# anonymous-author-918/deq-mpc-corl

Measured on AMD Instinct MI355X. Metric: QP solves/sec at (B,T=20,nx=13,nu=4), higher is better.
Workload: dtype f32

## Files before the change

### deq-mpc-corl_amd/_lib.py

```python
from __future__ import annotations

import ctypes as C
import os

_HERE = os.path.dirname(os.path.abspath(__file__))
LIB_PATH = os.environ.get("MI_ALQP_LIB") or os.path.join(_HERE, "csrc", "libmi_alqp.so")

ABI_VERSION = 16


class AlqpDims(C.Structure):
    _fields_ = [("B", C.c_int), ("T", C.c_int), ("nx", C.c_int), ("nu", C.c_int)]


class AlqpParams(C.Structure):
    _fields_ = [("al_iter", C.c_int), ("max_newton", C.c_int), ("n_ls", C.c_int),
                ("flags", C.c_int), ("rho_scale", C.c_double), ("variant", C.c_int),
                ("skip_flag", C.c_void_p), ("exit_tol", C.c_double), ("newton_counts", C.c_void_p),
                ("exit_scratch", C.c_void_p), ("quad_stagger", C.c_int)]


class AlqpTrace(C.Structure):
    _fields_ = [("g", C.c_void_p), ("d", C.c_void_p), ("phi", C.c_void_p),
                ("phi_prev", C.c_void_p), ("k", C.c_void_p), ("accept", C.c_void_p)]


class AlqpObstacles(C.Structure):
    _fields_ = [("pos", C.c_void_p), ("radius", C.c_double), ("nobs", C.c_int), ("state_estimator", C.c_int)]


class AlqpBwdDyn(C.Structure):
    _fields_ = [("lam", C.c_void_p), ("sb_lam", C.c_long), ("dF", C.c_void_p), ("dc", C.c_void_p), ("dx0", C.c_void_p)]


class AlqpIpmParams(C.Structure):
    _fields_ = [("flags", C.c_int), ("max_iter", C.c_int), ("iter0", C.c_int), ("kkt_eps", C.c_double),
                ("variant", C.c_int)]


class AlqpRigidParams(C.Structure):
    _fields_ = [("mass", C.c_double), ("J", C.c_double * 9), ("Jinv", C.c_double * 9), ("g", C.c_double * 3),
                ("motor_dist", C.c_double), ("kf", C.c_double), ("bf", C.c_double), ("km", C.c_double),
                ("act_scale", C.c_double), ("u_hover", C.c_double), ("pend_L", C.c_double), ("ss", C.c_double * 12),
                ("bf_force", C.c_double)]


IPM_VARIANTS = {"auto": 0, "generic_lds": 1, "generic_ws": 2, "resident": 3}


ALQP_IPM_INIT, ALQP_IPM_RESID, ALQP_IPM_STEP, ALQP_IPM_LOOP, ALQP_IPM_FINAL = 1, 2, 4, 8, 16
ALQP_INIT_MERIT = 1
ALQP_DUAL_UPDATE = 2
ALQP_SAVE_FACTOR = 4
ALQP_WS_PRIMED = 8
ALQP_EXIT_IN_KERNEL = 16
ALQP_E_COOP = -4
VARIANT_AUTO, VARIANT_TEAM, VARIANT_QUAD = 0, 1, 2

ERRORS = {-1: "bad argument", -2: "unsupported (nx, nu), or horizon / batch beyond what the requested kernel can hold or address",
          -3: "kernel launch failed", -4: "grid too large for a cooperative launch"}

_P = C.c_void_p
_SIGS = {
    "alqp_solve_nonlin": (C.c_int, [C.POINTER(AlqpDims), C.POINTER(AlqpParams), C.c_int, C.c_double, _P, _P, _P, _P, _P,
                                    C.c_long, C.c_long, _P, _P, _P, _P, _P, _P, _P, _P, C.c_size_t, _P]),
    "alqp_dyn_pendulum1l": (C.c_int, [C.c_long, _P, _P, C.c_double, _P, _P, _P, _P]),
    "alqp_dyn_cartpole1l": (C.c_int, [C.c_long, _P, _P, C.c_double, _P, _P, _P, _P]),
    "alqp_dyn_cartpole1l_v2": (C.c_int, [C.c_long, _P, _P, C.c_double, _P, _P, _P, _P]),
    "alqp_dyn_cartpole2l": (C.c_int, [C.c_long, _P, _P, C.c_double, _P, _P, _P, _P]),
    "alqp_dyn_rexquadrotor": (C.c_int, [C.c_long, C.POINTER(AlqpRigidParams), _P, _P, C.c_double, _P, _P, _P]),
    "alqp_dyn_flyingcartpole": (C.c_int, [C.c_long, C.POINTER(AlqpRigidParams), _P, _P, C.c_double, _P, _P, _P]),
    "alqp_solve_lin": (C.c_int, [C.POINTER(AlqpDims), C.POINTER(AlqpParams), _P, _P, _P, _P, _P, _P, _P,
                                 C.c_long, C.c_long, _P, _P, _P, _P, _P, _P, _P, _P,
                                 C.POINTER(AlqpTrace), _P, C.c_size_t, _P]),
    "alqp_solve_lin_shared": (C.c_int, [C.POINTER(AlqpDims), C.POINTER(AlqpParams), _P, _P, _P, _P,
                                        C.c_long, C.c_long, C.c_long, C.c_long, _P, _P, _P,
                                        C.c_long, C.c_long, _P, _P, _P, _P, _P, _P, _P, _P,
                                        C.POINTER(AlqpTrace), _P, C.c_size_t, _P]),
    "alqp_solve_lin_dense": (C.c_int, [C.POINTER(AlqpDims), C.POINTER(AlqpParams), _P, _P, _P, _P, _P, _P, _P,
                                       C.c_long, C.c_long, _P, _P, _P, _P, _P, _P, _P, _P,
                                       C.POINTER(AlqpTrace), _P]),
    "alqp_solve_lin_xbox": (C.c_int, [C.POINTER(AlqpDims), C.POINTER(AlqpParams), _P, _P, _P, _P, _P, _P, _P,
                                      C.c_long, C.c_long, _P, _P, C.c_long, C.c_long, _P, _P, _P, _P, _P, _P, _P, _P,
                                      C.POINTER(AlqpTrace), _P]),
    "alqp_solve_lin_poly": (C.c_int, [C.POINTER(AlqpDims), C.POINTER(AlqpParams), _P, _P, _P, _P, _P, _P, _P,
                                      C.c_long, C.c_long, _P, _P, C.c_int, C.c_long, C.c_long, C.c_long, C.c_long,
                                      _P, _P, _P, _P, _P, _P, _P, _P, C.POINTER(AlqpTrace), _P]),
    "alqp_newton_step": (C.c_int, [C.POINTER(AlqpDims), _P, _P, _P, _P, _P, _P, _P, _P, _P, _P,
                                   C.c_long, C.c_long, C.POINTER(AlqpObstacles), _P, C.c_size_t, _P, _P, _P, _P, _P]),
    "alqp_merit": (C.c_int, [C.POINTER(AlqpDims), C.c_int, _P, _P, _P, _P, _P, _P, _P, _P, _P,
                             C.c_long, C.c_long, C.POINTER(AlqpObstacles), _P, _P, _P]),
    "alqp_linesearch_pick": (C.c_int, [C.POINTER(AlqpDims), C.c_int, _P, _P, _P, _P, _P, _P, _P]),
    "alqp_dual_update": (C.c_int, [C.POINTER(AlqpDims), _P, _P, _P, _P, _P, C.c_long, C.c_long,
                                   C.POINTER(AlqpObstacles), _P, _P, C.c_double, _P]),
    "alqp_backward": (C.c_int, [C.POINTER(AlqpDims), _P, _P, C.c_size_t, _P, _P, _P, _P, _P, _P,
                                C.POINTER(AlqpBwdDyn), _P]),
    "alqp_merit_pick": (C.c_int, [C.POINTER(AlqpDims), C.c_int, _P, _P, _P, _P, _P, _P, _P, _P, _P,
                                  C.c_long, C.c_long, C.POINTER(AlqpObstacles), _P, _P, _P, _P, _P, _P, _P]),
    "alqp_ipm_solve": (C.c_int, [C.POINTER(AlqpDims), C.POINTER(AlqpIpmParams), _P, _P, _P, _P, _P, _P, _P,
                                 C.c_long, C.c_long, C.c_long, C.c_long, C.c_long, C.c_long, _P, C.c_size_t, _P,
                                 _P, _P, _P, _P, _P, _P, _P, _P, _P, _P]),
    "alqp_ipm_backward": (C.c_int, [C.POINTER(AlqpDims), _P, _P, C.c_long, C.c_long, C.c_long, C.c_long, _P, _P, _P,
                                    _P, C.c_size_t, _P, _P, _P, _P, C.c_int, _P]),
}
_PLAIN = {
    "alqp_abi_version": (C.c_int, []),
    "alqp_supported": (C.c_int, [C.POINTER(AlqpDims), C.c_int]),
    "alqp_supported_variant": (C.c_int, [C.POINTER(AlqpDims), C.c_int, C.c_int]),
# ... 42 lines not shown
```

### deq-mpc-corl_amd/backend.py

```python
from __future__ import annotations

import ctypes as C

import os

import torch

from . import _lib


def _dt(t):
    if t.dtype == torch.float32:
        return "f32"
    if t.dtype == torch.float64:
        return "f64"
    raise TypeError(f"mi_alqp: unsupported dtype {t.dtype}")


def _ptr(t, name, dtype=None, allow_none=False):
    if t is None:
        if allow_none:
            return None
        raise ValueError(f"mi_alqp: {name} is required")
    if not t.is_cuda:
        raise RuntimeError(
            f"mi_alqp: {name} lives on {t.device}; the solver only runs on a ROCm device "
            "(no CPU fallback)")
    if not t.is_contiguous():
        raise ValueError(f"mi_alqp: {name} must be contiguous")
    if dtype is not None and t.dtype != dtype:
        raise TypeError(f"mi_alqp: {name} has dtype {t.dtype}, expected {dtype}")
    return C.c_void_p(t.data_ptr())


def _stream():
    return C.c_void_p(torch.cuda.current_stream().cuda_stream)


_DEBUG_FLAGS = ((int(os.environ.get("ALQP_DEBUG_STAGGER", "0")) & 0xff) << 24) | ((int(os.environ.get("ALQP_DEBUG_STAGGER_CU", "0")) & 0xf) << 20)


class DynGrads:

    __slots__ = ("lam", "dF", "dc", "dx0")

    def __init__(self, lam=None, dF=None, dc=None, dx0=None):
        self.lam, self.dF, self.dc, self.dx0 = lam, dF, dc, dx0


def _dyn_args(dyn, dims, dt):
    if dyn is None:
        return None
    B, T, nx, nu = dims
    lam = dyn.lam
    if lam is None:
        if dyn.dF is not None:
            raise ValueError("mi_alqp: dyn.dF needs dyn.lam (the multipliers the solve returned)")
        lam_p, sb = None, 0
    else:
        if (not lam.is_cuda or lam.dtype != dt or lam.dim() != 2 or lam.shape[0] != B or lam.shape[1] < (T - 1) * nx
                or lam.stride(1) != 1 or (B > 1 and lam.stride(0) < (T - 1) * nx)):
            raise ValueError(f"mi_alqp: dyn.lam must be a [B, >= (T-1) nx] {dt} device tensor with unit inner stride")
        lam_p, sb = lam.data_ptr(), max(int(lam.stride(0)), (T - 1) * nx)
    outs = []
    for t, name, shape in ((dyn.dF, "dF", (B, T - 1, nx, nx + nu)), (dyn.dc, "dc", (B, T - 1, nx)),
                           (dyn.dx0, "dx0", (B, nx))):
        if t is not None and tuple(t.shape) != shape:
            raise ValueError(f"mi_alqp: dyn.{name} has shape {tuple(t.shape)}, expected {shape}")
        outs.append(None if t is None else _ptr(t, "dyn." + name, dt).value)
    return _lib.AlqpBwdDyn(lam_p, sb, *outs)


def _step_length(h, K, dt):
    if not torch.is_tensor(h):
        return float(h), None
    hpt = h.to(dt).reshape(-1).contiguous()
    if hpt.numel() != K:
        raise ValueError("mi_alqp: h must be a number or one value per point")
    return 0.0, hpt


class HipBackend:

    name = "hip"
    supports_exit_in_kernel = True
    default_variant = "auto"
    QUAD_MIN_BATCH = 4096

    def __init__(self):
        self.lib = _lib.load()
        self._ws = {}
        if os.environ.get("ALQP_QUAD_STAGGER") is not None:
# ... 520 lines not shown
```

### deq-mpc-corl_amd/csrc/alqp_quad.hip

```cpp
#if defined(ALQP_BWD_DYN_UNIT) || defined(ALQP_SHDYN_UNIT)
#undef ALQP_PHASE_TIMING
#endif
#include <hip/hip_runtime.h>

#include "alqp_quad.hpp"
#include "alqp_dims.hpp"
#include "alqp_launch.hpp"

#if defined(ALQP_QUAD_F32) == defined(ALQP_QUAD_F64)
#error "compile alqp_quad.hip with exactly one of -DALQP_QUAD_F32, -DALQP_QUAD_F64"
#endif

namespace alqp {

#ifndef ALQP_FUSE_LS
#define ALQP_FUSE_LS 1
#endif
#ifdef ALQP_PHASE_TIMING
__device__ unsigned long long g_phase_cycles[10];
#define QSTAMP(b) qd.stamp(b)
#else
#define QSTAMP(b)
#endif
#ifdef ALQP_SHDYN_UNIT
// ... 18 lines not shown
        int stag = a.stagger;
        const int mode = (a.flags >> 20) & 0xf;
        if ((a.flags >> 24) & 0xff) stag = (a.flags >> 24) & 0xff;
        if (stag > 0) {
            const unsigned hw = __builtin_amdgcn_s_getreg(4 | (0 << 6) | (31 << 11));
            int simd = (hw >> 4) & 3;
            if (mode == 1) simd = simd * 16 + ((hw >> 8) & 0xf);
            if (mode == 2) simd &= 1;
            if (mode == 3) simd = blockIdx.x & 1;
            if (mode == 4) simd = (simd & 1) ^ (blockIdx.x & 1);
            if (mode == 5) simd = (hw >> 8) & 3;
            for (int i = 0; i < simd * stag; ++i) __builtin_amdgcn_s_sleep(16);
        }
    }
#ifdef ALQP_ALIAS_ALL
    const int b = (active ? b_raw : a.B - 1) % ALQP_ALIAS_ALL;
#else
    const int b = active ? b_raw : a.B - 1;
#endif
    const int T = a.T, M = C::M(T);

    Quad<real, NX, NU> qd;
    __shared__ real w_lds[QCfg<real, NX, NU>::WLDS_WORDS];
    qd.wl = w_lds + threadIdx.x;
    qd.q = lane & 3;
    qd.T = T;
    qd.active = active;
    qd.gQd = a.Qd + (size_t)b * T * N;
    qd.gq = a.q + (size_t)b * T * N;
#ifdef ALQP_SHDYN_UNIT
    qd.gF = a.F + (size_t)b * a.sb_F;
    qd.gc = a.c + (size_t)b * a.sb_c;
    qd.mt_F = a.mt_F; qd.mt_c = a.mt_c;
#else
    qd.gF = a.F + (size_t)b * (T - 1) * NX * N;
    qd.gc = a.c + (size_t)b * (T - 1) * NX;
#endif
    qd.gx0 = a.x0 + (size_t)b * NX;
    qd.gulo = a.ulo + (size_t)b * a.sb_u;
    qd.guhi = a.uhi + (size_t)b * a.sb_u;
    qd.st_u = a.st_u;
    qd.gz = a.z + (size_t)b * T * N;
    qd.glam = a.lam + (size_t)b * M;
    qd.rec = ws + C::rec_base(b, T);
    qd.gFw = const_cast<real *>(qd.gF);
    qd.dyn_h = a.dyn_h;
    qd.rho = a.rho[b];
    qd.info = 0;
    real phi_prev = a.phi[b];
#ifdef ALQP_PHASE_TIMING
    for (int i = 0; i < 10; ++i) qd.tacc[i] = 0;
#endif
    QSTAMP(-1);
    if (!(a.flags & ALQP_WS_PRIMED)) {
        if constexpr (NL) qd.stage_in(false, false);
        else qd.stage_in(a.max_newton == 0 || a.al_iter == 0 || (a.flags & ALQP_EXIT_IN_KERNEL) ||
                         (!C::PHI0_FWD && (a.flags & ALQP_INIT_MERIT)));
    }
    const bool ref_exit = (a.flags & ALQP_EXIT_IN_KERNEL) != 0;
    int gphase = 0;

    int step_id = 0;
    bool pend = false;
    real alpha_pend = 0;
    int bad = 0;
    real rn2 = 0, phi_next = 0;
    for (int it = 0; it < a.al_iter; ++it) {
        bool phi_from_forward = false;
        if (a.flags & ALQP_INIT_MERIT) {
            if (it > 0) {
                phi_prev = phi_next;
            } else if (C::PHI0_FWD && a.max_newton > 0 && !ref_exit) {
                phi_from_forward = true;
            } else {
                if constexpr (NL) qd.template linearize<Dyn>(real(0), false);
                real p1[1];
                qd.template merit_candidates<1>(p1, true);
                phi_prev = p1[0];
            }
        }
        pend = false;
        double nrm_old = 0;
        int n_done = 0;
        if (ref_exit) {
            int bad0 = 0;
            const real r0 = it == 0 ? qd.rplus2(bad0) : rn2;
            nrm_old = sqrt(grid_sum_ordered(wave_sum_leaders(exit_term(r0, qor(qd.info)), active && qd.q == 0), a.exit_scratch, gphase));
        }
        for (int st = 0; st < a.max_newton; ++st, ++step_id) {
            real *tg = nullptr;
            if constexpr (TRACE) tg = (tr.g && active) ? tr.g + ((size_t)step_id * a.B + b) * T * N : nullptr;
            QSTAMP(9);
            if constexpr (NL) {
                qd.template linearize<Dyn>(alpha_pend, pend);
                pend = false;
            }
            qd.forward(tg, alpha_pend, pend, (phi_from_forward && st == 0) ? &phi_prev : nullptr);
            real ph[20];
            qd.template backward<FUSE_LS>(ph);
            QSTAMP(-1);
            if constexpr (TRACE) {
                if (tr.d && active) {
                    real *td = tr.d + ((size_t)step_id * a.B + b) * T * N;
                    for (int t = 0; t < T; ++t)
                        for (int j = qd.q; j < N; j += 4) td[t * N + j] = qd.recp(t)[C::wn(C::oY, j)];
                }
            }
            if constexpr (NL) qd.template merit_nonlin<Dyn>(ph);
            else if constexpr (!FUSE_LS) qd.template merit_candidates<20>(ph, false);
            QSTAMP(6);
            int kbest = 0;
            real best = ph[0];
#pragma unroll
            for (int k = 1; k < 20; ++k) {
                if (k < a.n_ls && !(best != best) && (ph[k] != ph[k] || ph[k] < best)) {
                    best = ph[k];
                    kbest = k;
                }
            }
            const bool acc = best < phi_prev;
            if constexpr (TRACE) {
                if (active && qd.q == 0) {
                    if (tr.phi)
#pragma unroll
                        for (int k = 0; k < 20; ++k)
                            if (k < a.n_ls) tr.phi[((size_t)step_id * a.n_ls + k) * a.B + b] = ph[k];
                    if (tr.phi_prev) tr.phi_prev[(size_t)step_id * a.B + b] = phi_prev;
                    if (tr.k) tr.k[(size_t)step_id * a.B + b] = kbest;
                    if (tr.accept) tr.accept[(size_t)step_id * a.B + b] = acc ? 1 : 0;
                }
            }
            const real alpha = acc ? real(1) / real(1 << kbest) : real(0);
            pend = true;
            alpha_pend = alpha;
            QSTAMP(7);
            phi_prev = best;
            if (ref_exit) {
                int bad1 = 0;
                real ph_unused = 0, r1 = 0;
                qd.template iter_end<Dyn>(alpha_pend, pend, false, (real)a.rho_scale, false, ph_unused, r1, bad1);
                pend = false;
                const double nw = sqrt(grid_sum_ordered(wave_sum_leaders(exit_term(r1, qor(qd.info)), active && qd.q == 0), a.exit_scratch, gphase));
                ++n_done;
                if (nw < a.exit_tol || fabs(nrm_old - nw) / nw < a.exit_tol) break;
                nrm_old = nw;
            }
        }
        if (ref_exit && a.newton_counts && blockIdx.x == 0 && lane == 0) a.newton_counts[it] = grid_barrier_timed_out(a.exit_scratch) ? -1 : n_done;
        bad = 0;
        qd.template iter_end<Dyn>(alpha_pend, pend, (a.flags & ALQP_DUAL_UPDATE) != 0, (real)a.rho_scale, it + 1 == a.al_iter,
                    phi_next, rn2, bad);
        pend = false;
    }
    if (a.al_iter <= 0) {
        rn2 = qd.rplus2(bad);
        qd.stage_out();
    }
#ifdef ALQP_PHASE_TIMING
    QSTAMP(9);
    if (lane == 0)
        for (int i = 0; i < 10; ++i) atomicAdd(&g_phase_cycles[i], qd.tacc[i]);
#endif
    if (active && qd.q == 0) {
        a.rho[b] = qd.rho;
        a.phi[b] = phi_prev;
        if (a.rnorm2) a.rnorm2[b] = rn2;
        if (a.info && qd.info && a.info[b] == 0) a.info[b] = qd.info;
        if (a.status) a.status[b] = bad ? 0 : 1;
    }
}

template <typename real, int NX, int NU, bool DYN = false>
__global__ __launch_bounds__(64) __attribute__((amdgpu_waves_per_eu(1, 1))) void k_backward_quad(BwdArgs<real, DYN> a, real *ws) {
    using C = QCfg<real, NX, NU>;
    constexpr int N = C::N;
    const int lane = threadIdx.x, qi = lane >> 2;
    const int b_raw = blockIdx.x * 16 + qi;
    const bool active = b_raw < a.B;
    const int b = active ? b_raw : a.B - 1;
    const int T = a.T;
    Quad<real, NX, NU> qd;
    __shared__ real w_lds[QCfg<real, NX, NU>::WLDS_WORDS];
    qd.wl = w_lds + threadIdx.x;
    qd.q = lane & 3;
    qd.T = T;
    qd.active = active;
    qd.gF = a.F + (size_t)b * (T - 1) * NX * N;
    qd.gQd = nullptr; qd.gq = nullptr; qd.gc = nullptr; qd.gx0 = nullptr; qd.gulo = nullptr; qd.guhi = nullptr;
    qd.st_u = 0;
    qd.gz = nullptr; qd.glam = nullptr;
    qd.rec = ws + C::rec_base(b, T);
    qd.rho = a.rho[b];
    qd.info = 0;
    qd.solve_forward(a.gbar + (size_t)b * T * N);
    real unused[20];
    qd.template backward<false>(unused);
    if (active) {
        const real *zf = a.z_final + (size_t)b * T * N;
        real *qg = a.q_grad + (size_t)b * T * N;
        real *Qg = a.Qd_grad + (size_t)b * T * N;
        for (int t = 0; t < T; ++t)
// ... 182 lines not shown
```

### deq-mpc-corl_amd/csrc/alqp_quad.hpp

```cpp
#pragma once
#include <hip/hip_runtime.h>

#include <type_traits>

#include "alqp_team.hpp"
#include "alqp_dyn.hpp"

namespace alqp {

template <int Q>
__device__ inline float qb(float v) {
    return __builtin_bit_cast(float, __builtin_amdgcn_mov_dpp(__builtin_bit_cast(int, v), Q * 0x55, 0xF, 0xF, true));
}
template <int Q>
__device__ inline double qb(double v) {
    long long b = __builtin_bit_cast(long long, v);
    int lo = __builtin_amdgcn_mov_dpp((int)(b & 0xffffffffll), Q * 0x55, 0xF, 0xF, true);
    int hi = __builtin_amdgcn_mov_dpp((int)(b >> 32), Q * 0x55, 0xF, 0xF, true);
    return __builtin_bit_cast(double, ((long long)hi << 32) | (unsigned int)lo);
}
template <typename real>
__device__ inline real qbv(real v, int src) {
    switch (src & 3) {
        case 0: return qb<0>(v);
// ... 42 lines not shown
}
__device__ inline void gst4(float *p, float a, float b, float c, float d) {
    f4u t; t.x = a; t.y = b; t.z = c; t.w = d;
    *reinterpret_cast<f4u *>(p) = t;
}
__device__ inline void gst4(double *p, double a, double b, double c, double d) {
    d4u t; t.x = a; t.y = b; t.z = c; t.w = d;
    *reinterpret_cast<d4u *>(p) = t;
}
template <int LEN, typename real>
__device__ inline void gload(const real *p, real (&dst)[LEN]) {
#pragma unroll
    for (int c = 0; c + 4 <= LEN; c += 4) gld4(p + c, dst[c], dst[c + 1], dst[c + 2], dst[c + 3]);
#pragma unroll
    for (int c = (LEN / 4) * 4; c < LEN; ++c) dst[c] = p[c];
}

#ifndef ALQP_W_LDS
#define ALQP_W_LDS 1
#endif
#ifndef ALQP_EXP_NOQ
#define ALQP_EXP_NOQ 0
#endif
#ifndef ALQP_EXP_NORS
#define ALQP_EXP_NORS 0
#endif
#ifndef ALQP_EXP_NOL
#define ALQP_EXP_NOL 0
#endif
template <typename real, int SW, int N, bool IN_LDS>
struct WPanel {
    real a[SW][N];
    __device__ __forceinline__ real (&operator[](int s))[N] { return a[s]; }
    __device__ __forceinline__ const real (&operator[](int s) const)[N] { return a[s]; }
};
template <typename real, int N>
struct WRowLds {
    real *p;
    __device__ __forceinline__ real &operator[](int k) const { return p[k * 64]; }
};
template <typename real, int SW, int N>
struct WPanel<real, SW, N, true> {
    real *base;
    __device__ __forceinline__ WRowLds<real, N> operator[](int s) const { return WRowLds<real, N>{base + s * N * 64}; }
};
template <int LEN, typename real>
__device__ __forceinline__ void gload(const real *p, WRowLds<real, LEN> row) {
    real tmp[LEN];
    gload<LEN>(p, tmp);
#pragma unroll
    for (int k = 0; k < LEN; ++k) row[k] = tmp[k];
}

struct NoDyn {
    static constexpr int ID = 0;
};

struct Fld {
    int h, t;
};
template <int H, int T>
struct FldT {
    static constexpr int h = H, t = T;
    __host__ __device__ constexpr operator Fld() const { return {H, T}; }
};
template <typename real>
struct FRef {
    real *p;
    Fld f;
};
template <typename real, int H, int T>
__device__ __forceinline__ FRef<std::remove_const_t<real>> operator+(real *p, FldT<H, T>) {
    return {const_cast<std::remove_const_t<real> *>(p), Fld{H, T}};
}

template <typename real, int NX_, int NU_>
struct QCfg {
    static constexpr int NX = NX_, NU = NU_, N = NX_ + NU_;
    static constexpr int SH = (N + 3) / 4;
    static constexpr int SW = (NX + 3) / 4;
    static constexpr int SY = SH;
    static constexpr int HT = 2 * SH * (SH + 1);
    __host__ __device__ static constexpr int hidx(int s, int j) { return 2 * s * (s + 1) + j; }
    static constexpr int ST = 2 * SW * (SW + 1);
    static constexpr int BLK = 64 / (int)sizeof(real);
#ifndef ALQP_REC_IL_F32
#define ALQP_REC_IL_F32 2
#endif
    static constexpr int IL = sizeof(real) == 4 ? ALQP_REC_IL_F32 : 1;
    static_assert(IL == 1 || BLK == 16, "groups of 16 words are 64-byte blocks");
    __host__ __device__ static constexpr int w(int x) { return (x / 16) * (16 * IL) + x % 16; }
    static constexpr int NLAST = N - 4 * (SH - 1);
    __host__ __device__ static constexpr int lanes_of(int s) { return s == SH - 1 ? NLAST : 4; }
    __host__ __device__ static constexpr int lstride(int s) { return lanes_of(s) == 3 ? 16 : 4 * lanes_of(s); }
    __host__ __device__ static constexpr int lbase(int s) {
        int o = 0;
        for (int i = 0; i < s; ++i) o += (i + 1) * lstride(i);
        return o;
    }
    static constexpr int LW = lbase(SH);
    static constexpr bool PHI0_FWD = sizeof(real) == 4;
#ifndef ALQP_S_AFTER_F32
#define ALQP_S_AFTER_F32 0
#endif
    static constexpr bool S_AFTER = sizeof(real) == 8 || ALQP_S_AFTER_F32;
#ifndef ALQP_W_LDS_F32
// ... 399 lines not shown
        const real a0 = sel4(real(1), real(0.5), real(0.25), real(0.125), q);
        for (int t = 0; t < T; ++t) {
            const bool dyn = t < T - 1;
            const real *rp = recp(t), *rn = recp(dyn ? t + 1 : t);
            real zt[N], dt[N], Qt[N], qt[N], zn[NX], dn[NX], le[NX], lu[NU], ll[NU], bu[NU], bl[NU];
            ld_rep_n(rp + C::oZ, zt);
            ld_rep_n(rp + C::oY, dt);
            ld_rep_n(rp + C::oQ, Qt);
            ld_rep_n(rp + C::oq, qt);
            ld_repx_of_n(rn + C::oZ, zn);
            ld_repx_of_n(rn + C::oY, dn);
            ld_rep_x(rp + C::oLE, le);
            ld_rep_us(rp, lu, ll, bu, bl);
            real alpha = a0;
#pragma unroll
            for (int i = 0; i < 5; ++i) {
                real zc[N];
                real acc = 0;
#pragma unroll
                for (int j = 0; j < N; ++j) {
                    zc[j] = fma_(alpha, dt[j], zt[j]);
                    acc = fma_(fma_(real(0.5) * Qt[j], zc[j], qt[j]), zc[j], acc);
                }
#pragma unroll
                for (int ju = 0; ju < NU; ++ju) {
                    const real vu = zc[NX + ju] - bu[ju], vl = bl[ju] - zc[NX + ju];
                    const real cu = fmax_(vu, real(0)), cl = fmax_(vl, real(0));
                    acc += fma_(lu[ju], vu, ll[ju] * vl) + real(0.5) * rho * fma_(cu, cu, cl * cl);
                }
                if (dyn) {
                    real xn[NX];
                    dyn_value<Dyn, real>(zc, dyn_h, xn);
#pragma unroll
                    for (int r = 0; r < NX; ++r) {
                        const real rr = fma_(alpha, dn[r], zn[r]) - xn[r];
                        acc = fma_(fma_(real(0.5) * rho, rr, le[r]), rr, acc);
                    }
                }
                if (t == 0) {
#pragma unroll
                    for (int r = 0; r < NX; ++r) {
                        const real rr = zc[r] - x0v[r];
                        acc = fma_(fma_(real(0.5) * rho, rr, li[r]), rr, acc);
                    }
                }
                m[i] += acc;
                alpha *= real(0.0625);
            }
        }
#pragma unroll
        for (int k = 0; k < 20; ++k) phi[k] = qbv(m[k >> 2], k);
    }

    template <bool EXT = false>
    __device__ __forceinline__ void forward(real *g_out, real alpha, bool pending, real *phi0, const real *gxn = nullptr) {
        real mdist = 0;
        real S[ST], Sy[SW];
        real vpo[SW], Syo[SW];
#pragma unroll
        for (int i = 0; i < ST; ++i) S[i] = 0;
#pragma unroll
        for (int s = 0; s < SW; ++s) Sy[s] = 0;
        {
            real z0[SW], xi[SW], li[SW], r0[SW];
            if constexpr (EXT) {
                ld_own_ext<NX>(gz, z0);
                ld_own_ext<NX>(glam + (T - 1) * NX, li);
            } else {
                ld_ownx_of_n(recp(0) + C::oZ, z0);
                ld_own_x(recp(T - 1) + C::oLE, li);
            }
            ld_own_ext<NX>(gx0, xi);
            if (pending) {
                real d0[SW];
                ld_ownx_of_n(recp(0) + C::oY, d0);
#pragma unroll
                for (int s = 0; s < SW; ++s) z0[s] = fma_(alpha, d0[s], z0[s]);
            }
#pragma unroll
            for (int s = 0; s < SW; ++s) {
                bool valid = 4 * s + 3 < NX || 4 * s + q < NX;
                if constexpr (EXT) valid = valid && !no_init;
                const real r = valid ? z0[s] - xi[s] : real(0);
                vpo[s] = valid ? fma_(rho, r, li[s]) : real(0);
                if constexpr (C::PHI0_FWD) mdist += valid ? fma_(fma_(real(0.5) * rho, r, li[s]), r, real(0)) : real(0);
                Syo[s] = 0;
                r0[s] = r;
            }
            if (!EXT && active) st_own_x(recp(T - 1) + C::oR, r0);
        }
        for (int t = 0; t < T; ++t) {
            const bool dyn = t < T - 1;
            WT W = wpanel();
            real Y[N];
            real dio[SY];
            real v[SW];
            real zs[SY];
            real hob[3] = {0, 0, 0};
            real *rp = recp(t);
            {
                real zt[N];
                real Qo[SY], qo[SY];
                real cs[SW], zn[SW], lm[SW];
                real lu, ll, bu, bl;
                const int td = dyn ? t : (T > 1 ? T - 2 : 0);
                const real *rn = recp(td + 1);
                if constexpr (EXT) {
                    ld_own_ext<N>(gz + t * N, zs);
                    ld_own_ext<N>(gQd + t * N, Qo);
                    ld_own_ext<N>(gq + t * N, qo);
                    load_F_rows(td, W);
                    ld_own_ext<NX>(gxn + td * NX, cs);
                    ld_own_ext<NX>(gz + (td + 1) * N, zn);
                    ld_own_ext<NX>(glam + td * NX, lm);
                    const int ju = own_ju(), jc = ju < NU ? ju : 0;
                    const real *lb = glam + T * NX + t * (2 * NU + nobs);
                    const bool has = ju < NU;
                    lu = has ? lb[jc] : real(0);
                    ll = has ? lb[NU + jc] : real(0);
                    bu = has ? guhi[t * st_u + jc] : real(0);
                    bl = has ? gulo[t * st_u + jc] : real(0);
                } else {
                    ld_own_n(rp + C::oZ, zs);
                    if constexpr (ALQP_EXP_NOQ) { for (int m = 0; m < SY; ++m) Qo[m] = real(1); }
                    else ld_own_n(rp + C::oQ, Qo);
                    ld_own_n(rp + C::oq, qo);
                    load_F_rows(td, W);
                    ld_own_x(rp + C::oC, cs);
                    ld_ownx_of_n(rn + C::oZ, zn);
                    ld_own_x(rp + C::oLE, lm);
                    ld_own_us(rp, lu, ll, bu, bl);
                }
                if (pending) {
                    real dt[SY], dn[SW];
                    ld_own_n(rp + C::oY, dt);
                    ld_ownx_of_n(rn + C::oY, dn);
#pragma unroll
                    for (int m = 0; m < SY; ++m) zs[m] = fma_(alpha, dt[m], zs[m]);
#pragma unroll
                    for (int s = 0; s < SW; ++s) zn[s] = fma_(alpha, dn[s], zn[s]);
                }
                ALQP_STAMP(0);
#pragma unroll
                for (int k = 0; k < N; ++k) zt[k] = qbv(zs[k >> 2], k);
                real rro[SW];
                if (!dyn) {
#pragma unroll
                    for (int s = 0; s < SW; ++s)
#pragma unroll
                        for (int k = 0; k < N; ++k) W[s][k] = 0;
                }
#pragma unroll
                for (int s = 0; s < SW; ++s) {
                    const int r = 4 * s + q;
                    real xn = cs[s];
                    if constexpr (!EXT) {
#pragma unroll
                        for (int k = 0; k < N; ++k) xn = fma_(W[s][k], zt[k], xn);
                    }
                    const real rr = zn[s] - xn;
                    const bool ok = dyn && r < NX;
                    v[s] = ok ? fma_(rho, rr, lm[s]) : real(0);
                    rro[s] = ok ? rr : real(0);
                    if constexpr (C::PHI0_FWD) mdist += ok ? fma_(fma_(real(0.5) * rho, rr, lm[s]), rr, real(0)) : real(0);
                }
                if (!ALQP_EXP_NORS && !EXT && dyn && active) st_own_x(rp + C::oR, rro);
                constexpr int MU0 = NX / 4;
                real zu = 0;
#pragma unroll
                for (int m = MU0; m < SY; ++m) zu = (4 * m + q >= NX && 4 * m + q < N) ? zs[m] : zu;
                const real vu = zu - bu, vl = bl - zu;
                const real au = vu >= 0 ? real(1) : real(0), al = vl >= 0 ? real(1) : real(0);
                const real cu = fmax_(vu, real(0)), cl = fmax_(vl, real(0));
                const real gu = fma_(rho, cu, lu) - fma_(rho, cl, ll);
                const real du = rho * (au + al);
                if constexpr (C::PHI0_FWD)
                    mdist += own_ju() < NU ? fma_(lu, vu, ll * vl) + real(0.5) * rho * fma_(cu, cu, cl * cl) : real(0);
                real go[SY];
#pragma unroll
                for (int m = 0; m < SY; ++m) {
                    const int j = 4 * m + q;
                    const bool isx = (4 * m + 3 < NX) ? true : (4 * m >= NX ? false : j < NX);
                    const bool isu = (4 * m + 3 < NX) ? false : (j >= NX && j < N);
                    real g = fma_(Qo[m], zs[m], qo[m]);
                    real d = Qo[m];
                    if constexpr (C::PHI0_FWD) mdist = fma_(fma_(real(0.5) * Qo[m], zs[m], qo[m]), zs[m], mdist);
                    g += isx ? vpo[m < SW ? m : 0] : (isu ? gu : real(0));
                    bool pinned = isx;
                    if constexpr (EXT) {
                        pinned = isx && !(no_init && t == 0);
                        if (no_init && isu) g = 0;
                    }
                    d += pinned ? rho : (isu ? du : real(0));
                    dio[m] = d;
                    go[m] = g;
                }
                if constexpr (EXT && NX >= 3) {
                    if (nobs > 0) {
                        const real *lk = glam + T * NX + t * (2 * NU + nobs) + 2 * NU;
                        real gob = 0;
                        for (int k = 0; k < nobs; ++k) {
                            const real *o = gobs + (size_t)(t * nobs + k) * 3;
                            const real d0 = zt[0] - o[0], d1 = zt[1] - o[1], d2 = zt[2] - o[2];
                            const real ck = obs_r2 - fma_(d0, d0, fma_(d1, d1, d2 * d2));
                            const real dh = q == 0 ? d0 : (q == 1 ? d1 : d2);
                            gob = fma_(fma_(rho, ck > 0 ? ck : real(0), lk[k]), real(-2) * dh, gob);
                            if (ck >= 0) {
                                const real w4 = real(4) * rho * dh;
                                hob[0] = fma_(w4, d0, hob[0]); hob[1] = fma_(w4, d1, hob[1]); hob[2] = fma_(w4, d2, hob[2]);
                            }
                        }
                        go[0] += q < 3 ? gob : real(0);
                    }
                }
#pragma unroll
                for (int m = 0; m < SY; ++m) {
                    const bool isx = (4 * m + 3 < NX) ? true : (4 * m >= NX ? false : 4 * m + q < NX);
                    go[m] = -go[m] - (isx ? Syo[m < SW ? m : 0] : real(0));
                }
                real fv[N];
#pragma unroll
                for (int j = 0; j < N; ++j) {
                    real p = 0;
                    if (dyn) {
#pragma unroll
                        for (int s = 0; s < SW; ++s) p = fma_(W[s][j], v[s], p);
                        p = qsum(p);
                    }
                    fv[j] = p;
                    Y[j] = qbv(go[j >> 2], j) + p;
                }
                if (g_out) {
                    real fo[SY];
                    own_of<N, SY>(fv, fo);
#pragma unroll
                    for (int m = 0; m < SY; ++m) {
                        const bool isx = (4 * m + 3 < NX) ? true : (4 * m >= NX ? false : 4 * m + q < NX);
                        if (4 * m + 3 < N || 4 * m + q < N)
                            g_out[t * N + 4 * m + q] = -(go[m] + fo[m]) - (isx ? Syo[m < SW ? m : 0] : real(0));
// ... 95 lines not shown
                if constexpr (C::S_AFTER) ipv[j] = ip;
                if (!C::S_AFTER && dyn) {
#pragma unroll
                    for (int b = 0; b < NX; ++b) {
                        const real wbj = qbv(W[b >> 2][j], b) * ip;
#pragma unroll
                        for (int s = (b >> 2); s < SW; ++s) S[C::hidx(s, b)] = fma_(W[s][j], wbj, S[C::hidx(s, b)]);
                    }
                    const real yip = Y[j] * ip;
#pragma unroll
                    for (int s = 0; s < SW; ++s) Sy[s] = fma_(W[s][j], yip, Sy[s]);
                }
                H[C::hidx(j >> 2, j)] = (q == (j & 3)) ? ip : H[C::hidx(j >> 2, j)];
            }
            ALQP_STAMP(2);
            if (active) {
                if (!(ALQP_EXP_NOL && t >= T - ALQP_EXP_NOL))
#pragma unroll
                for (int s = 0; s < SH; ++s)
#pragma unroll
                    for (int c = 0; c <= s; ++c)
                        if (C::lanes_of(s) == 4 || q < C::lanes_of(s))
                            gst4(lchunk(rp, s, c, q), H[C::hidx(s, 4 * c)],
                                 H[C::hidx(s, 4 * c + 1)], H[C::hidx(s, 4 * c + 2)], H[C::hidx(s, 4 * c + 3)]);
                real yo[SY];
                own_of<N, SY>(Y, yo);
                st_own_n(rp + C::oY, yo);
                if (pending) st_own_n(rp + C::oZ, zs);
            }

            if constexpr (C::S_AFTER) {
                if (dyn) {
#pragma unroll
                    for (int j = 0; j < N; ++j) {
#pragma unroll
                        for (int b = 0; b < NX; ++b) {
                            const real wbj = qbv(W[b >> 2][j], b) * ipv[j];
#pragma unroll
                            for (int s = (b >> 2); s < SW; ++s) S[C::hidx(s, b)] = fma_(W[s][j], wbj, S[C::hidx(s, b)]);
                        }
                        const real yip = Y[j] * ipv[j];
#pragma unroll
                        for (int s = 0; s < SW; ++s) Sy[s] = fma_(W[s][j], yip, Sy[s]);
                    }
                }
            }
#pragma unroll
            for (int s = 0; s < SW; ++s) {
                vpo[s] = v[s];
                Syo[s] = Sy[s];
            }
            ALQP_STAMP(3);
        }
        if constexpr (C::PHI0_FWD) { if (phi0) *phi0 = qsum(mdist); }
    }

    __host__ __device__ static constexpr int lane_lo(int m, int j) { return m == (j >> 2) ? (j & 3) + 1 : 0; }
    __device__ __forceinline__ bool in_lanes(int lo, int hi) const {
        return lo == 0 ? q < hi : (hi == 4 ? q >= lo : (q >= lo && q < hi));
    }
    __device__ __forceinline__ void lsolve_own(const real (&H)[HT], real (&u)[SY]) const {
#pragma unroll
        for (int j = 0; j < N; ++j) {
            const int mj = j >> 2;
            const real wj = qbv(u[mj] * H[C::hidx(mj, j)], j);
#pragma unroll
            for (int m = mj; m < SH; ++m) {
                const int lo = lane_lo(m, j);
                if (lo >= C::lanes_of(m)) continue;
                const real v = fma_(-H[C::hidx(m, j)], wj, u[m]);
                u[m] = lo == 0 ? v : (q >= lo ? v : u[m]);
            }
        }
    }
    __device__ __forceinline__ void ltsolve_own(const real (&H)[HT], const real (&y)[SY], real (&d)[SY], real (&rep)[N]) const {
#pragma unroll
        for (int m = 0; m < SY; ++m) d[m] = 0;
#pragma unroll
        for (int i = N - 1; i >= 0; --i) {
            const int mi = i >> 2;
            real p = 0;
            bool any = false;
#pragma unroll
            for (int m = mi; m < SH; ++m) {
                const int lo = lane_lo(m, i), hi = C::lanes_of(m);
                if (lo >= hi) continue;
                const real h = (lo == 0 && hi == 4) ? H[C::hidx(m, i)] : (in_lanes(lo, hi) ? H[C::hidx(m, i)] : real(0));
                p = any ? fma_(h, d[m], p) : h * d[m];
                any = true;
            }
            real r = y[mi];
            if (any) r -= qsum(p);
            const real di = qbv(r * H[C::hidx(mi, i)], i);
            rep[i] = di;
            d[mi] = (q == (i & 3)) ? di : d[mi];
        }
    }

    template <bool LS>
    __device__ __forceinline__ void backward(real (&phi)[20], real *d_ext = nullptr) {
        constexpr int MU0 = NX / 4;
        real c0 = 0, c1 = 0, c2 = 0;
        real acc[20];
        real rvT[SW], lvT[SW];
#pragma unroll
        for (int k = 0; k < 20; ++k) acc[k] = 0;
#pragma unroll
        for (int s = 0; s < SW; ++s) rvT[s] = lvT[s] = 0;
        real dxs[SW];
#pragma unroll
        for (int s = 0; s < SW; ++s) dxs[s] = 0;
        for (int t = T - 1; t >= 0; --t) {
            const bool dyn = t < T - 1;
            real *rp = recp(t);
            real H[HT];
            if (ALQP_EXP_NOL && t >= T - ALQP_EXP_NOL) {
#pragma unroll
                for (int i = 0; i < HT; ++i) H[i] = real(1);
            } else
#pragma unroll
            for (int s = 0; s < SH; ++s)
#pragma unroll
                for (int c = 0; c <= s; ++c) {
                    const int ql = (C::lanes_of(s) == 4 || q < C::lanes_of(s)) ? q : 0;
                    gld4(lchunk(rp, s, c, ql), H[C::hidx(s, 4 * c)],
                         H[C::hidx(s, 4 * c + 1)], H[C::hidx(s, 4 * c + 2)], H[C::hidx(s, 4 * c + 3)]);
                }
            real yo[SY];
            ld_own_n(rp + C::oY, yo);
            WT W = wpanel();
            load_F_rows(dyn ? t : (T > 1 ? T - 2 : 0), W);
            real zz[SY], QQ[SY], qq[SY], rv[SW], lv[SW];
            real lu = 0, ll = 0, bu = 0, bl = 0;
            if constexpr (LS) {
                ld_own_n(rp + C::oZ, zz);
                if constexpr (ALQP_EXP_NOQ) { for (int m = 0; m < SY; ++m) QQ[m] = real(1); }
                else ld_own_n(rp + C::oQ, QQ);
                ld_own_n(rp + C::oq, qq);
                ld_own_us(rp, lu, ll, bu, bl);
                if constexpr (ALQP_EXP_NORS) { for (int s = 0; s < SW; ++s) rv[s] = real(0); }
                else ld_own_x(rp + C::oR, rv);
                ld_own_x(rp + C::oLE, lv);
            }
            ALQP_STAMP(4);
            if (dyn) {
                real vv[N];
#pragma unroll
                for (int j = 0; j < N; ++j) {
                    real p = 0;
#pragma unroll
                    for (int s = 0; s < SW; ++s) p = fma_(W[s][j], dxs[s], p);
                    vv[j] = qsum(p);
                }
                real uo[SY];
                own_of<N, SY>(vv, uo);
                lsolve_own(H, uo);
#pragma unroll
                for (int m = 0; m < SY; ++m) yo[m] = fma_(rho, uo[m], yo[m]);
            }
            real down[SY], Y[N];
            ltsolve_own(H, yo, down, Y);
            if (active) {
                if (d_ext) st_own_ext<N>(d_ext + t * N, down);
                else st_own_n(rp + C::oY, down);
            }
            real sv[SW];
#pragma unroll
            for (int s = 0; s < SW; ++s) sv[s] = 0;
            if (dyn) {
#pragma unroll
                for (int s = 0; s < SW; ++s) {
                    const int r = 4 * s + q;
                    real p = 0;
#pragma unroll
                    for (int k = 0; k < N; ++k) p = fma_(W[s][k], Y[k], p);
                    sv[s] = (4 * s + 3 < NX || r < NX) ? dxs[s] - p : real(0);
                }
                if (!ALQP_EXP_NORS && active && !d_ext) st_own_x(rp + C::oS, sv);
            }
            if constexpr (LS) {
                real zu = 0, du = 0;
#pragma unroll
                for (int m = 0; m < SY; ++m) {
                    const int j = 4 * m + q;
                    const real ok = (4 * m + 3 < N || j < N) ? real(1) : real(0);
                    const real z = zz[m], d = down[m], Qv = QQ[m] * ok, qv = qq[m] * ok;
                    c0 = fma_(fma_(real(0.5) * Qv, z, qv), z, c0);
                    c1 = fma_(fma_(Qv, z, qv), d, c1);
                    c2 = fma_(real(0.5) * Qv * d, d, c2);
                    if (m >= MU0) {
                        const bool mine = j >= NX && j < N;
                        zu = mine ? z : zu;
                        du = mine ? d : du;
                    }
                }
                {
                    const real isu = own_ju() < NU ? real(1) : real(0);
                    real alpha = 1;
#pragma unroll
                    for (int k = 0; k < 20; ++k) {
                        real zk = fma_(alpha, du, zu);
                        real vu = zk - bu, vl = bl - zk;
                        real cu = fmax_(vu, real(0)), cl = fmax_(vl, real(0));
                        acc[k] = fma_(isu, fma_(lu, vu, ll * vl) + real(0.5) * rho * fma_(cu, cu, cl * cl), acc[k]);
                        alpha *= real(0.5);
                    }
                }
                if (dyn) {
#pragma unroll
                    for (int s = 0; s < SW; ++s) {
                        const int r = 4 * s + q;
                        const real ok = (4 * s + 3 < NX || r < NX) ? real(1) : real(0);
                        const real rr = rv[s] * ok, ss = sv[s] * ok, lm = lv[s] * ok;
                        c0 = fma_(fma_(real(0.5) * rho, rr, lm), rr, c0);
                        c1 = fma_(fma_(rho, rr, lm), ss, c1);
                        c2 = fma_(real(0.5) * rho * ss, ss, c2);
                    }
                } else {
#pragma unroll
                    for (int s = 0; s < SW; ++s) {
                        rvT[s] = rv[s];
                        lvT[s] = lv[s];
                    }
                }
            }
#pragma unroll
            for (int s = 0; s < SW; ++s) dxs[s] = (4 * s + 3 < NX || 4 * s + q < NX) ? down[s] : real(0);
            ALQP_STAMP(5);
        }
        if (active && !d_ext) st_own_x(recp(T - 1) + C::oS, dxs);
        if constexpr (LS) {
#pragma unroll
            for (int s = 0; s < SW; ++s) {
                const int r = 4 * s + q;
                const real ok = (4 * s + 3 < NX || r < NX) ? real(1) : real(0);
                const real rr = rvT[s] * ok, ss = dxs[s], lm = lvT[s] * ok;
                c0 = fma_(fma_(real(0.5) * rho, rr, lm), rr, c0);
                c1 = fma_(fma_(rho, rr, lm), ss, c1);
                c2 = fma_(real(0.5) * rho * ss, ss, c2);
            }
            c0 = qsum(c0);
            c1 = qsum(c1);
            c2 = qsum(c2);
            real alpha = 1;
#pragma unroll
            for (int k = 0; k < 20; ++k) {
                phi[k] = qsum(acc[k]) + fma_(alpha, fma_(alpha, c2, c1), c0);
                alpha *= real(0.5);
            }
        }
    }

    __device__ __forceinline__ void solve_forward(const real *gbar) {
        real e[N];
#pragma unroll
        for (int j = 0; j < N; ++j) e[j] = 0;
        for (int t = 0; t < T; ++t) {
            real *rp = recp(t);
            real H[HT];
#pragma unroll
            for (int s = 0; s < SH; ++s)
#pragma unroll
                for (int c = 0; c <= s; ++c) {
                    const int ql = (C::lanes_of(s) == 4 || q < C::lanes_of(s)) ? q : 0;
                    gld4(lchunk(rp, s, c, ql), H[C::hidx(s, 4 * c)],
                         H[C::hidx(s, 4 * c + 1)], H[C::hidx(s, 4 * c + 2)], H[C::hidx(s, 4 * c + 3)]);
                }
            real yo[SY];
            ld_own_ext<N, SY>(gbar + t * N, yo);
            WT W = wpanel();
            load_F_rows(t > 0 ? t - 1 : 0, W);
#pragma unroll
            for (int m = 0; m < SY; ++m) yo[m] = -yo[m];
            if (t > 0) {
#pragma unroll
                for (int s = 0; s < SW; ++s) {
                    real p = 0;
#pragma unroll
                    for (int k = 0; k < N; ++k) p = fma_(W[s][k], e[k], p);
                    yo[s] = (4 * s + 3 < NX || 4 * s + q < NX) ? fma_(rho, p, yo[s]) : yo[s];
                }
            }
            lsolve_own(H, yo);
// ... 233 lines not shown
```

### include/mi_alqp.h

```cpp
#ifndef MI_ALQP_H
#define MI_ALQP_H

#include <stddef.h>

#ifdef __cplusplus
extern "C" {
#endif

typedef struct AlqpDims {
    int B;
    int T;
    int nx;
    int nu;
} AlqpDims;

typedef struct AlqpObstacles {
    const void *pos;
    double radius;
    int nobs;
    int state_estimator;
} AlqpObstacles;

#define ALQP_INIT_MERIT   1
#define ALQP_DUAL_UPDATE  2
#define ALQP_SAVE_FACTOR  4
#define ALQP_WS_PRIMED    8

#define ALQP_EXIT_IN_KERNEL 16

typedef struct AlqpParams {
    int al_iter;
    int max_newton;
    int n_ls;
    int flags;
    double rho_scale;
    int variant;
    const double *skip_flag;
    double exit_tol;
    int *newton_counts;
    double *exit_scratch;
    int quad_stagger;
} AlqpParams;

typedef struct AlqpTrace {
    void *g;
    void *d;
    void *phi;
    void *phi_prev;
    int *k;
    int *accept;
} AlqpTrace;

#define ALQP_E_BADARG     (-1)
#define ALQP_E_UNSUPPORTED (-2)
#define ALQP_E_LAUNCH     (-3)
#define ALQP_E_COOP       (-4)

int alqp_supported(const AlqpDims *dims, int is_f64);
int alqp_supported_variant(const AlqpDims *dims, int is_f64, int variant);
int alqp_pick_variant(const AlqpDims *dims, int is_f64, int flags, long quad_min_batch);
size_t alqp_lds_bytes(const AlqpDims *dims, int is_f64);
int alqp_qps_per_wave(const AlqpDims *dims, int is_f64);
size_t alqp_workspace_bytes(const AlqpDims *dims, int is_f64);

int alqp_solve_lin_f32(const AlqpDims *dims, const AlqpParams *prm, const void *Qd, const void *q,
                       const void *F, const void *c, const void *x0, const void *u_lo,
                       const void *u_hi, long sb_u, long st_u, void *z, void *lam, void *rho,
                       void *phi, void *rnorm2, int *info, unsigned char *status,
                       void *factor_out, const AlqpTrace *trace, void *workspace, size_t ws_bytes,
                       void *stream);
int alqp_solve_lin_f64(const AlqpDims *dims, const AlqpParams *prm, const void *Qd, const void *q,
                       const void *F, const void *c, const void *x0, const void *u_lo,
                       const void *u_hi, long sb_u, long st_u, void *z, void *lam, void *rho,
                       void *phi, void *rnorm2, int *info, unsigned char *status,
                       void *factor_out, const AlqpTrace *trace, void *workspace, size_t ws_bytes,
                       void *stream);

int alqp_solve_lin_shared_f32(const AlqpDims *dims, const AlqpParams *prm, const void *Qd, const void *q,
                              const void *F, const void *c, long sb_F, long st_F, long sb_c, long st_c,
                              const void *x0, const void *u_lo, const void *u_hi, long sb_u, long st_u, void *z,
                              void *lam, void *rho, void *phi, void *rnorm2, int *info, unsigned char *status,
// ... 182 lines not shown
```

Before: 6.185 million.

## Fuse input staging and dual update into the forward Riccati pass

Adds forward-pass modes that copy the problem data from the caller's arrays into the workspace records during the first forward sweep, and that apply the augmented-Lagrangian dual update and merit evaluation inside the next iteration's forward sweep. The separate stage-in pass and the iter_end pass between outer iterations are skipped. The backward pass now skips storing the step vector S when it is not needed. The aim is to remove whole passes over the workspace and the memory traffic they cost, in exchange for more complex forward code, extra register pressure, and a debug flag to turn the fusion off.

Result: no change. 6.314 million (median of 3 runs) (+2.1%).

```diff
diff --git a/deq-mpc-corl_amd/_lib.py b/deq-mpc-corl_amd/_lib.py
--- a/deq-mpc-corl_amd/_lib.py
+++ b/deq-mpc-corl_amd/_lib.py
@@ -54,6 +54,7 @@
 ALQP_SAVE_FACTOR = 4
 ALQP_WS_PRIMED = 8
 ALQP_EXIT_IN_KERNEL = 16
+ALQP_NO_PASS_FUSION = 32
 ALQP_E_COOP = -4
 VARIANT_AUTO, VARIANT_TEAM, VARIANT_QUAD = 0, 1, 2
 
diff --git a/deq-mpc-corl_amd/backend.py b/deq-mpc-corl_amd/backend.py
--- a/deq-mpc-corl_amd/backend.py
+++ b/deq-mpc-corl_amd/backend.py
@@ -38,6 +38,8 @@
 
 
 _DEBUG_FLAGS = ((int(os.environ.get("ALQP_DEBUG_STAGGER", "0")) & 0xff) << 24) | ((int(os.environ.get("ALQP_DEBUG_STAGGER_CU", "0")) & 0xf) << 20)
+if os.environ.get("ALQP_DEBUG_NO_PASS_FUSION", "0") not in ("", "0"):
+    _DEBUG_FLAGS |= _lib.ALQP_NO_PASS_FUSION
 
 
 class DynGrads:
diff --git a/deq-mpc-corl_amd/csrc/alqp_quad.hip b/deq-mpc-corl_amd/csrc/alqp_quad.hip
--- a/deq-mpc-corl_amd/csrc/alqp_quad.hip
+++ b/deq-mpc-corl_amd/csrc/alqp_quad.hip
@@ -94,12 +94,20 @@
     for (int i = 0; i < 10; ++i) qd.tacc[i] = 0;
 #endif
     QSTAMP(-1);
-    if (!(a.flags & ALQP_WS_PRIMED)) {
+    const bool ref_exit = (a.flags & ALQP_EXIT_IN_KERNEL) != 0;
+#ifndef ALQP_EXP_FUSE_PARTS
+#define ALQP_EXP_FUSE_PARTS 7
+#endif
+    constexpr bool CAN_FUSE = C::PHI0_FWD && !NL;
+    const bool fuse = CAN_FUSE && !(a.flags & ALQP_NO_PASS_FUSION) && !ref_exit && a.max_newton > 0 && a.al_iter > 0;
+    const bool copy_in_fwd = fuse && (ALQP_EXP_FUSE_PARTS & 1) && !(a.flags & ALQP_WS_PRIMED);
+    const bool dual_in_fwd = fuse && (ALQP_EXP_FUSE_PARTS & 2);
+    const bool s_on_demand = fuse && (ALQP_EXP_FUSE_PARTS & 4);
+    if (!(a.flags & ALQP_WS_PRIMED) && !copy_in_fwd) {
         if constexpr (NL) qd.stage_in(false, false);
         else qd.stage_in(a.max_newton == 0 || a.al_iter == 0 || (a.flags & ALQP_EXIT_IN_KERNEL) ||
                          (!C::PHI0_FWD && (a.flags & ALQP_INIT_MERIT)));
     }
-    const bool ref_exit = (a.flags & ALQP_EXIT_IN_KERNEL) != 0;
     int gphase = 0;
 
     int step_id = 0;
@@ -107,6 +115,15 @@
     real alpha_pend = 0;
     int bad = 0;
     real rn2 = 0, phi_next = 0;
+    bool fwd_done = false;
+    if constexpr (CAN_FUSE) {
+        if (copy_in_fwd) {
+            real *tg = nullptr;
+            if constexpr (TRACE) tg = (tr.g && active) ? tr.g + (size_t)b * T * N : nullptr;
+            qd.template forward<false, FW_COPYIN>(tg, real(0), false, (a.flags & ALQP_INIT_MERIT) ? &phi_prev : nullptr);
+            fwd_done = true;
+        }
+    }
     for (int it = 0; it < a.al_iter; ++it) {
         bool phi_from_forward = false;
         if (a.flags & ALQP_INIT_MERIT) {
@@ -137,9 +154,21 @@
                 qd.template linearize<Dyn>(alpha_pend, pend);
                 pend = false;
             }
-            qd.forward(tg, alpha_pend, pend, (phi_from_forward && st == 0) ? &phi_prev : nullptr);
+            bool plain = true;
+            if constexpr (CAN_FUSE) {
+                if (fwd_done) {
+                    fwd_done = false;
+                    plain = false;
+                } else if (st == 0 && it > 0 && dual_in_fwd) {
+                    qd.template forward<false, FW_DUAL>(tg, alpha_pend, true, &phi_next, nullptr,
+                                                        (a.flags & ALQP_DUAL_UPDATE) != 0, (real)a.rho_scale);
+                    if (a.flags & ALQP_INIT_MERIT) phi_prev = phi_next;
+                    plain = false;
+                }
+            }
+            if (plain) qd.forward(tg, alpha_pend, pend, (phi_from_forward && st == 0) ? &phi_prev : nullptr);
             real ph[20];
-            qd.template backward<FUSE_LS>(ph);
+            qd.template backward<FUSE_LS>(ph, nullptr, TRACE || !s_on_demand || st + 1 == a.max_newton);
             QSTAMP(-1);
             if constexpr (TRACE) {
                 if (tr.d && active) {
@@ -189,6 +218,7 @@
             }
         }
         if (ref_exit && a.newton_counts && blockIdx.x == 0 && lane == 0) a.newton_counts[it] = grid_barrier_timed_out(a.exit_scratch) ? -1 : n_done;
+        if (dual_in_fwd && it + 1 < a.al_iter) continue;
         bad = 0;
         qd.template iter_end<Dyn>(alpha_pend, pend, (a.flags & ALQP_DUAL_UPDATE) != 0, (real)a.rho_scale, it + 1 == a.al_iter,
                     phi_next, rn2, bad);
diff --git a/deq-mpc-corl_amd/csrc/alqp_quad.hpp b/deq-mpc-corl_amd/csrc/alqp_quad.hpp
--- a/deq-mpc-corl_amd/csrc/alqp_quad.hpp
+++ b/deq-mpc-corl_amd/csrc/alqp_quad.hpp
@@ -118,6 +118,8 @@
     for (int k = 0; k < LEN; ++k) row[k] = tmp[k];
 }
 
+constexpr int FW_PLAIN = 0, FW_COPYIN = 1, FW_DUAL = 2;
+
 struct NoDyn {
     static constexpr int ID = 0;
 };
@@ -623,9 +625,18 @@
         for (int k = 0; k < 20; ++k) phi[k] = qbv(m[k >> 2], k);
     }
 
-    template <bool EXT = false>
-    __device__ __forceinline__ void forward(real *g_out, real alpha, bool pending, real *phi0, const real *gxn = nullptr) {
+    template <bool EXT = false, int MODE = FW_PLAIN>
+    __device__ __forceinline__ void forward(real *g_out, real alpha, bool pending, real *phi0, const real *gxn = nullptr,
+                                            bool dual = false, real rho_scale = real(1)) {
+        static_assert(!EXT || MODE == FW_PLAIN, "the caller-mode step has no record to fill or update");
+        constexpr bool CIN = MODE == FW_COPYIN, DUP = MODE == FW_DUAL;
+        constexpr bool MERIT = C::PHI0_FWD && !DUP;
+        if constexpr (DUP) pending = true;
         real mdist = 0;
+        real pc0 = 0, pacc0 = 0;
+        const real rho_o = rho;
+        real rnT[DUP ? SW : 1];
+        if constexpr (DUP) { if (dual) rho = rho * rho_scale; }
         real S[ST], Sy[SW];
         real vpo[SW], Syo[SW];
 #pragma unroll
@@ -634,7 +645,7 @@
         for (int s = 0; s < SW; ++s) Sy[s] = 0;
         {
             real z0[SW], xi[SW], li[SW], r0[SW];
-            if constexpr (EXT) {
+            if constexpr (EXT || CIN) {
                 ld_own_ext<NX>(gz, z0);
                 ld_own_ext<NX>(glam + (T - 1) * NX, li);
             } else {
@@ -642,6 +653,21 @@
                 ld_own_x(recp(T - 1) + C::oLE, li);
             }
             ld_own_ext<NX>(gx0, xi);
+            if constexpr (DUP) {
+                real rT[SW], sT[SW];
+                ld_own_x(recp(T - 1) + C::oR, rT);
+                ld_own_x(recp(T - 1) + C::oS, sT);
+#pragma unroll
+                for (int s = 0; s < SW; ++s) {
+                    const bool valid = 4 * s + 3 < NX || 4 * s + q < NX;
+                    real rn = fma_(alpha, sT[s], rT[s]);
+                    if (!valid) rn = 0;
+                    rnT[s] = rn;
+                    const real ln = valid ? (dual ? fma_(rho_o, rn, li[s]) : li[s]) : real(0);
+                    if (dual) li[s] = ln;
+                }
+                if (dual && active) st_own_x(recp(T - 1) + C::oLE, li);
+            }
             if (pending) {
                 real d0[SW];
                 ld_ownx_of_n(recp(0) + C::oY, d0);
@@ -654,7 +680,7 @@
                 if constexpr (EXT) valid = valid && !no_init;
                 const real r = valid ? z0[s] - xi[s] : real(0);
                 vpo[s] = valid ? fma_(rho, r, li[s]) : real(0);
-                if constexpr (C::PHI0_FWD) mdist += valid ? fma_(fma_(real(0.5) * rho, r, li[s]), r, real(0)) : real(0);
+                if constexpr (MERIT) mdist += valid ? fma_(fma_(real(0.5) * rho, r, li[s]), r, real(0)) : real(0);
                 Syo[s] = 0;
                 r0[s] = r;
             }
@@ -691,6 +717,33 @@
                     ll = has ? lb[NU + jc] : real(0);
                     bu = has ? guhi[t * st_u + jc] : real(0);
                     bl = has ? gulo[t * st_u + jc] : real(0);
+                } else if constexpr (CIN) {
+                    ld_own_ext<N>(gz + t * N, zs);
+                    ld_own_ext<N>(gQd + t * N, Qo);
+                    ld_own_ext<N>(gq + t * N, qo);
+                    load_F_rows(td, W);
+                    ld_own_ext<NX>(gc + ALQP_C_STAGE(td), cs);
+                    ld_own_ext<NX>(gz + (td + 1) * N, zn);
+                    ld_own_ext<NX>(glam + t * NX, lm);
+                    const int ju = own_ju(), jc = ju < NU ? ju : 0;
+                    const real *lb = glam + T * NX + t * 2 * NU;
+                    const bool has = ju < NU;
+                    lu = has ? lb[jc] : real(0);
+                    ll = has ? lb[NU + jc] : real(0);
+                    bu = has ? guhi[t * st_u + jc] : real(0);
+                    bl = has ? gulo[t * st_u + jc] : real(0);
+                    if (!dyn) {
+#pragma unroll
+                        for (int s = 0; s < SW; ++s) cs[s] = 0;
+                    }
+                    if (active) {
+                        st_own_n(rp + C::oZ, zs);
+                        st_own_n(rp + C::oQ, Qo);
+                        st_own_n(rp + C::oq, qo);
+                        st_own_x(rp + C::oLE, lm);
+                        st_own_us(rp, lu, ll, bu, bl);
+                        st_own_x(rp + C::oC, cs);
+                    }
                 } else {
                     ld_own_n(rp + C::oZ, zs);
                     if constexpr (ALQP_EXP_NOQ) { for (int m = 0; m < SY; ++m) Qo[m] = real(1); }
@@ -702,6 +755,11 @@
                     ld_own_x(rp + C::oLE, lm);
                     ld_own_us(rp, lu, ll, bu, bl);
                 }
+                real rvo[DUP ? SW : 1], svo[DUP ? SW : 1];
+                if constexpr (DUP) {
+                    ld_own_x(rp + C::oR, rvo);
+                    ld_own_x(rp + C::oS, svo);
+                }
                 if (pending) {
                     real dt[SY], dn[SW];
                     ld_own_n(rp + C::oY, dt);
@@ -712,6 +770,18 @@
                     for (int s = 0; s < SW; ++s) zn[s] = fma_(alpha, dn[s], zn[s]);
                 }
                 ALQP_STAMP(0);
+                if constexpr (DUP) {
+#pragma unroll
+                    for (int m = 0; m < SY; ++m) {
+                        const int j = 4 * m + q;
+                        const bool valid = 4 * m + 3 < N || j < N;
+                        const real ok = valid ? real(1) : real(0);
+                        const real z = valid ? zs[m] : real(0);
+                        const real Qv = Qo[m] * ok, qv = qo[m] * ok;
+                        zs[m] = z;
+                        pc0 = fma_(fma_(real(0.5) * Qv, z, qv), z, pc0);
+                    }
+                }
 #pragma unroll
                 for (int k = 0; k < N; ++k) zt[k] = qbv(zs[k >> 2], k);
                 real rro[SW];
@@ -720,6 +790,21 @@
                     for (int s = 0; s < SW; ++s)
 #pragma unroll
                         for (int k = 0; k < N; ++k) W[s][k] = 0;
+                }
+                if constexpr (DUP) {
+#pragma unroll
+                    for (int s = 0; s < SW; ++s) {
+                        const int r = 4 * s + q;
+                        const bool valid = 4 * s + 3 < NX || r < NX;
+                        const real ok = valid ? real(1) : real(0);
+                        real rn = dyn ? fma_(alpha, svo[s], rvo[s]) : rnT[s];
+                        if (!valid) rn = 0;
+                        const real ln = valid ? ((dual && dyn) ? fma_(rho_o, rn, lm[s]) : lm[s]) : real(0);
+                        const real rr = rn * ok, lmm = ln * ok;
+                        pc0 = fma_(fma_(real(0.5) * rho, rr, lmm), rr, pc0);
+                        if (dual) lm[s] = ln;
+                    }
+                    if (dual && dyn && active) st_own_x(rp + C::oLE, lm);
                 }
 #pragma unroll
                 for (int s = 0; s < SW; ++s) {
@@ -733,7 +818,7 @@
                     const bool ok = dyn && r < NX;
                     v[s] = ok ? fma_(rho, rr, lm[s]) : real(0);
                     rro[s] = ok ? rr : real(0);
-                    if constexpr (C::PHI0_FWD) mdist += ok ? fma_(fma_(real(0.5) * rho, rr, lm[s]), rr, real(0)) : real(0);
+                    if constexpr (MERIT) mdist += ok ? fma_(fma_(real(0.5) * rho, rr, lm[s]), rr, real(0)) : real(0);
                 }
                 if (!ALQP_EXP_NORS && !EXT && dyn && active) st_own_x(rp + C::oR, rro);
                 constexpr int MU0 = NX / 4;
@@ -743,9 +828,25 @@
                 const real vu = zu - bu, vl = bl - zu;
                 const real au = vu >= 0 ? real(1) : real(0), al = vl >= 0 ? real(1) : real(0);
                 const real cu = fmax_(vu, real(0)), cl = fmax_(vl, real(0));
+                if constexpr (DUP) {
+                    const bool isub = own_ju() < NU;
+                    const real isu = isub ? real(1) : real(0);
+                    real lun = lu, lln = ll;
+                    if (dual) {
+                        const real a = fma_(rho_o, vu, lu), c = fma_(rho_o, vl, ll);
+                        lun = a < 0 ? real(0) : a;
+                        lln = c < 0 ? real(0) : c;
+                    }
+                    if (isub && active) {
+                        if (dual) st_own_us(rp, lun, lln, bu, bl);
+                    }
+                    pacc0 = fma_(isu, fma_(lun, vu, lln * vl) + real(0.5) * rho * fma_(cu, cu, cl * cl), pacc0);
+                    lu = isub ? lun : lu;
+                    ll = isub ? lln : ll;
+                }
                 const real gu = fma_(rho, cu, lu) - fma_(rho, cl, ll);
                 const real du = rho * (au + al);
-                if constexpr (C::PHI0_FWD)
+                if constexpr (MERIT)
                     mdist += own_ju() < NU ? fma_(lu, vu, ll * vl) + real(0.5) * rho * fma_(cu, cu, cl * cl) : real(0);
                 real go[SY];
 #pragma unroll
@@ -755,7 +856,7 @@
                     const bool isu = (4 * m + 3 < NX) ? false : (j >= NX && j < N);
                     real g = fma_(Qo[m], zs[m], qo[m]);
                     real d = Qo[m];
-                    if constexpr (C::PHI0_FWD) mdist = fma_(fma_(real(0.5) * Qo[m], zs[m], qo[m]), zs[m], mdist);
+                    if constexpr (MERIT) mdist = fma_(fma_(real(0.5) * Qo[m], zs[m], qo[m]), zs[m], mdist);
                     g += isx ? vpo[m < SW ? m : 0] : (isu ? gu : real(0));
                     bool pinned = isx;
                     if constexpr (EXT) {
@@ -957,7 +1058,11 @@
             }
             ALQP_STAMP(3);
         }
-        if constexpr (C::PHI0_FWD) { if (phi0) *phi0 = qsum(mdist); }
+        if constexpr (MERIT) { if (phi0) *phi0 = qsum(mdist); }
+        if constexpr (DUP) {
+            pc0 = qsum(pc0);
+            *phi0 = qsum(pacc0) + pc0;
+        }
     }
 
     __host__ __device__ static constexpr int lane_lo(int m, int j) { return m == (j >> 2) ? (j & 3) + 1 : 0; }
@@ -1003,7 +1108,7 @@
     }
 
     template <bool LS>
-    __device__ __forceinline__ void backward(real (&phi)[20], real *d_ext = nullptr) {
+    __device__ __forceinline__ void backward(real (&phi)[20], real *d_ext = nullptr, bool keep_s = true) {
         constexpr int MU0 = NX / 4;
         real c0 = 0, c1 = 0, c2 = 0;
         real acc[20];
@@ -1081,7 +1186,7 @@
                     for (int k = 0; k < N; ++k) p = fma_(W[s][k], Y[k], p);
                     sv[s] = (4 * s + 3 < NX || r < NX) ? dxs[s] - p : real(0);
                 }
-                if (!ALQP_EXP_NORS && active && !d_ext) st_own_x(rp + C::oS, sv);
+                if (!ALQP_EXP_NORS && active && !d_ext && keep_s) st_own_x(rp + C::oS, sv);
             }
             if constexpr (LS) {
                 real zu = 0, du = 0;
@@ -1133,7 +1238,7 @@
             for (int s = 0; s < SW; ++s) dxs[s] = (4 * s + 3 < NX || 4 * s + q < NX) ? down[s] : real(0);
             ALQP_STAMP(5);
         }
-        if (active && !d_ext) st_own_x(recp(T - 1) + C::oS, dxs);
+        if (active && !d_ext && keep_s) st_own_x(recp(T - 1) + C::oS, dxs);
         if constexpr (LS) {
 #pragma unroll
             for (int s = 0; s < SW; ++s) {
diff --git a/include/mi_alqp.h b/include/mi_alqp.h
--- a/include/mi_alqp.h
+++ b/include/mi_alqp.h
@@ -27,6 +27,7 @@
 #define ALQP_WS_PRIMED    8
 
 #define ALQP_EXIT_IN_KERNEL 16
+#define ALQP_NO_PASS_FUSION 32
 
 typedef struct AlqpParams {
     int al_iter;
```
